# Yachim/schwarzschild-raytracer

Hardware: AMD Instinct MI355X
Metric: Mpixels/s at 1920x1080, 2000 geodesic steps; 1/2/4/8 MI355X (higher is better)
Workload: dtype f32

## Files before the change

### schwarzschild-raytracer_amd/csrc/kernels/geodesic.hip

```cpp
#include <hip/hip_runtime.h>

#include <cstdint>
#include <type_traits>

typedef float sr_v4f __attribute__((ext_vector_type(4)));
typedef const __attribute__((address_space(4))) sr_v4f sr_cfloat4;
__device__ __forceinline__ float4 ldc(const sr_cfloat4* p) {
    const sr_v4f v = *p;
    return make_float4(v.x, v.y, v.z, v.w);
}

#include "../device_scene.h"

namespace {

#define SR_PI 3.1415926535f
#define SR_EPS 0.0000001f

struct f2 { float x, y; };
struct f3 { float x, y, z; };
struct f4 { float x, y, z, w; };
struct m3 { f3 c0, c1, c2; };

__device__ __forceinline__ f2 F2(float x, float y) { f2 r; r.x = x; r.y = y; return r; }
// ... 283 lines not shown
            c = fminf(c - qm, SR_BUDGET_TMAX);
        }
    }
    return c - 1.8f * slot_mu(sl) * a;
}
__device__ __forceinline__ float clearance_bh(float a) {
    return (fabsf(a - 1.0f) - SR_MU_QUADRATIC * 3.0f) - 1.8f * SR_MU_QUADRATIC * a;
}
__device__ __forceinline__ bool outward_clear(float cn, float br, float mu, float qk, float pl1, float a, float dip) {
    const float S = __builtin_fmaf(0.01f * a, a, __builtin_fmaf(2.0f, a, 1.0f));
    const float Sc = S + pl1;
    return a * dip > (cn + br + __builtin_fmaf(mu, S, qk * Sc * Sc)) * 1.001f;
}
__device__ __forceinline__ float plane_window(const sr_dev_slot& sl, f3 A, f3 B, float a, float perr, float dphi) {
    const f3 dv = B - A;
    const f3 nrm_ = ld3(sl.a1);
    const float y = dot(B - ld3(sl.pos), nrm_);
    const float len = __builtin_amdgcn_sqrtf(dot(dv, dv));
    if (!(len > 1e-6f) || !(len < 0.5f * a) || !(a > 1.0f)) return 0.0f;
    const float il = __builtin_amdgcn_rcpf(len);
    const float a2 = a * a;
    const float kap = 6.06f * __builtin_amdgcn_rcpf(a2);
    const float c = (y > 0.0f ? -1.0f : 1.0f) * dot(dv, nrm_) * il;
    const float th0 = __builtin_fmaf(kap, len, __builtin_fmaf(2.0f * perr, il, 1e-4f));
    const float m = (sl.mp + sl.mu * __builtin_fmaf(3.1f, a, 1.0f)) * 1.001f + perr;
    const float R = fabsf(y) - m;
    if (!(R > 0.0f)) return 0.0f;
    const float b = c + th0;
    const float L = (__builtin_amdgcn_sqrtf(__builtin_fmaf(b, b, 2.0f * kap * R)) - b) * (a2 * (1.0f / 6.06f));
    const float ch = 1.5f * a * dphi;
    const float Lc = fminf(L, fminf(__builtin_fmaf(0.5f, a, -ch), (1.5f - th0) * (a2 * (1.0f / 6.06f)) - ch));
    const float th1 = __builtin_fmaf(kap, Lc, th0);
    const float f = 1.0f - (th1 * th1 + th1 * th0 + th0 * th0) * (1.0f / 6.0f);
    return (Lc > 0.0f && f > 0.0f) ? Lc * f * 0.998f : 0.0f;
}
#ifndef SR_INIT_WINDOW
#define SR_INIT_WINDOW 1
#endif
struct PlaneWinCam {
    bool ok;
    f3 wn;
    float k2r;
    float kap, a2s, cap;
};
__device__ __forceinline__ PlaneWinCam plane_window_cam(const sr_dev_slot& sl, f3 A, float a, float perr, float dphi) {
    PlaneWinCam w;
    w.ok = false;
    w.wn = F3(0.0f, 0.0f, 0.0f);
    w.k2r = w.kap = w.a2s = w.cap = 0.0f;
    const f3 nrm_ = ld3(sl.a1);
    const float y = dot(A - ld3(sl.pos), nrm_);
    if (!(a > 1.0f)) return w;
    const float a2 = a * a;
    const float kap = 6.06f * __builtin_amdgcn_rcpf(a2);
    w.wn = nrm_ * (y > 0.0f ? -1.0f : 1.0f);
    const float th0 = 1e-4f;
    const float m = (sl.mp + sl.mu * __builtin_fmaf(3.1f, a, 1.0f)) * 1.001f + perr;
    const float R = fabsf(y) - m;
    if (!(R > 0.0f)) return w;
    w.k2r = 2.0f * kap * R;
    w.kap = kap;
    w.a2s = a2 * (1.0f / 6.06f);
    const float ch = 1.5f * a * dphi;
    w.cap = fminf(__builtin_fmaf(0.5f, a, -ch), (1.5f - th0) * (a2 * (1.0f / 6.06f)) - ch);
    w.ok = true;
    return w;
}
__device__ __forceinline__ float plane_window_dir(f3 wn, float k2r, float kap, float a2s, float cap, f3 d) {
    const float c = dot(d, wn);
    const float th0 = 1e-4f;
    const float b = c + th0;
    const float L = (__builtin_amdgcn_sqrtf(__builtin_fmaf(b, b, k2r)) - b) * a2s;
    const float Lc = fminf(L, cap);
    const float th1 = __builtin_fmaf(kap, Lc, th0);
    const float f = 1.0f - (th1 * th1 + th1 * th0 + th0 * th0) * (1.0f / 6.0f);
    return (Lc > 0.0f && f > 0.0f) ? Lc * f * 0.998f : 0.0f;
}
#ifndef SR_OUT_CYL_CM
#define SR_OUT_CYL_CM 1
#endif
#ifndef SR_OUT_FAR
#define SR_OUT_FAR 1
#endif
__device__ __forceinline__ bool outward_slot(const sr_dev_slot& sl, bool cyl_par, float a, float dip) {
    if (SR_OUT_CYL_CM) cyl_par = false;
    if (sl.type == SR_OBJECT_PLANE || (sl.type == SR_OBJECT_CYLINDER && (cyl_par || !(sl.x1 > 0.0f)))) return false;
    if (SR_OUT_FAR)
        return outward_clear(sl.rf, 0.0f, slot_mu(sl), sl.type == SR_OBJECT_CYLINDER ? sl.qk : 0.0f, sl.pl1, a, dip);
    return outward_clear(sl.cn, sl.br, sl.mu, sl.type == SR_OBJECT_CYLINDER ? sl.qk : 0.0f, sl.pl1, a, dip);
}

#define SR_PIN(x) asm volatile("" : "+s"(x))
__device__ __forceinline__ sr_dev_slot pin_slot(const sr_dev_slot& g) {
    sr_dev_slot sl = g;
    SR_PIN(sl.type);
    SR_PIN(sl.rb);
    SR_PIN(sl.mp);
    SR_PIN(sl.br);
    SR_PIN(sl.mu);
    SR_PIN(sl.pl1);
    SR_PIN(sl.qk);
    SR_PIN(sl.bc[0]);
    SR_PIN(sl.bc[1]);
    SR_PIN(sl.bc[2]);
    SR_PIN(sl.x0);
    SR_PIN(sl.pos[0]);
    SR_PIN(sl.pos[1]);
    SR_PIN(sl.pos[2]);
    SR_PIN(sl.x1);
    SR_PIN(sl.a0[0]);
    SR_PIN(sl.a0[1]);
    SR_PIN(sl.a0[2]);
    SR_PIN(sl.x2);
    SR_PIN(sl.a1[0]);
    SR_PIN(sl.a1[1]);
    SR_PIN(sl.a1[2]);
    SR_PIN(sl.a2[0]);
    SR_PIN(sl.a2[1]);
    SR_PIN(sl.a2[2]);
    return sl;
}

__device__ __forceinline__ float clearance_slab(const sr_dev_slot& sl, f3 A, float a) {
    if (!(sl.mp < INFINITY)) return -INFINITY;
    const float y = dot(A - ld3(sl.pos), ld3(sl.a1));
    const float ey = fmaxf(0.0f, fmaxf(-y, y - sl.x0));
    return ey - sl.mp - 1.8f * SR_MU_QUADRATIC * a;
}

__device__ __forceinline__ float nmin(float m, float e) { return __builtin_elementwise_minimum(m, e); }

#ifndef SR_WG
#define SR_WG 64
#endif
#define SR_WG_PER_TILE (256 / SR_WG)
#define SR_E_STRIDE SR_WG
#ifndef SR_NC_KERNEL
#define SR_NC_KERNEL 0
#endif
#ifndef SR_AHEAD
#define SR_AHEAD 2.0f
#endif
#ifndef SR_FAST_UNROLL
#define SR_FAST_UNROLL SR_FAST_UNROLL_DEFAULT
#endif
#ifndef SR_AHEAD_T
#define SR_AHEAD_T 1.0f
#endif
#ifndef SR_CM_ITER
#define SR_CM_ITER 1
#endif
#ifndef SR_COAST
#define SR_COAST 1
#endif
template <int NB, int NC, bool TR = false>
struct BudgetLayout {
    static constexpr int PA0 = NB + 1;
    static constexpr int SLAB0 = PA0 + 2 * NC;
    static constexpr int BT = SLAB0 + NC;
    static constexpr int BM = BT + 1, BCX = BT + 2, BCY = BT + 3, BMH = BT + 4, BCM = BT + 5, BUHI = BT + 6;
    static constexpr int BTR = BT + 7;
    static constexpr int ROWS = BT + 7 + (TR ? 1 : 0);
};
#define SR_REACH_TR (1u << 30)
#ifndef SR_BH_WINDOW
#define SR_BH_WINDOW 1
#endif
#define SR_BH_U 0.986f
#define SR_U_NOWIN 0x1.93e592p+99f
#define SR_BH_RWIN 1.0143f
#ifndef SR_BH_WINDOW2
#define SR_BH_WINDOW2 1
#endif
#define SR_BH_ULO2 0.90910f
#define SR_BH_RMAX2 1.0999f
#define SR_BH_DIP2 0.9995f
#define SR_BH_DIP 0.9935f

__device__ __forceinline__ float ball_q(float R, float cx, float cy) {
    if (!(R < INFINITY)) return R == INFINITY ? -INFINITY : INFINITY;
    const float c = fabsf(cx) + fabsf(cy);
    const float Rt = R * (1.0f / 1.0101f) - 3.0e-6f * (c + R);
    if (!(Rt > 0.0f)) return INFINITY;
    const float s = c + Rt;
    return __builtin_fmaf(2.0e-6f * s, s, (cx * cx + cy * cy) - Rt * Rt);
}

template <int NB_, int NC_, bool TR_ = false>
struct Budget {
    using L = BudgetLayout<NB_, NC_, TR_>;
    static constexpr int NB = NB_, NC = NC_;
    static constexpr bool TR = TR_;
    float* E;
    __device__ __forceinline__ float ld(int row) const { return E[row * SR_E_STRIDE]; }
    __device__ __forceinline__ void st(int row, float v) const { E[row * SR_E_STRIDE] = v; }
    __device__ __forceinline__ float T() const { return ld(L::BT); }
    __device__ __forceinline__ void setT(float v) const { st(L::BT, v); }
    __device__ __forceinline__ float m() const { return ld(L::BM); }
    __device__ __forceinline__ void setM(float v) const { st(L::BM, v); }
    __device__ __forceinline__ float cx() const { return ld(L::BCX); }
    __device__ __forceinline__ float cy() const { return ld(L::BCY); }
    __device__ __forceinline__ void setC(float x, float y) const {
        st(L::BCX, x);
        st(L::BCY, y);
    }
    __device__ __forceinline__ float mh() const { return ld(L::BMH); }
    __device__ __forceinline__ void setMh(float v) const { st(L::BMH, v); }
    __device__ __forceinline__ uint32_t cm() const { return __float_as_uint(ld(L::BCM)) & 0xffu; }
    __device__ __forceinline__ uint32_t excl() const { return __float_as_uint(ld(L::BCM)) >> 8; }
    __device__ __forceinline__ void setCm(uint32_t cm, uint32_t excl) const {
        st(L::BCM, __uint_as_float(cm | (excl << 8)));
    }
    __device__ __forceinline__ float etr() const { return ld(L::BTR); }
    __device__ __forceinline__ void setEtr(float v) const { st(L::BTR, v); }
    __device__ __forceinline__ float uhi() const { return ld(L::BUHI); }
    __device__ __forceinline__ void setUhi(float v) const { st(L::BUHI, v); }
    static __device__ __forceinline__ bool inner(float uhi) { return uhi > SR_BH_U && uhi < 1.0f; }
    static __device__ __forceinline__ float ulo_of(float uhi, float u_f) { return inner(uhi) ? SR_BH_ULO2 : u_f; }
    SR_PROBE_BUDGET_FIELDS
};

__device__ __forceinline__ float xplane_need(const sr_dev_slot& sl, float xs) {
    if (sl.type == SR_OBJECT_PLANE || sl.type == SR_OBJECT_CYLINDER) return INFINITY;
    return (sl.br + sl.mu * xs) * 1.001f + 1.0e-4f + 1.0e-5f * sl.cn;
}
__device__ __forceinline__ uint32_t plane_off_bit(f3 bc, int j, f3 n, float nn, float need) {
    const float h = dot(bc, n);
    return (uint32_t)(h * h > (need * need) * (nn * 1.0002f)) << j;
}
__device__ __forceinline__ uint32_t xplane_bit(const sr_dev_slot& sl, int j, f3 n, float nn, float xs) {
    return plane_off_bit(ld3(sl.bc), j, n, nn, xplane_need(sl, xs));
}
#ifndef SR_XCYL
#define SR_XCYL 1
#endif
__device__ __forceinline__ uint32_t xcyl_bit(const sr_dev_slot& sl, int j, f3 n, float nn, float need) {
    return plane_off_bit(ld3(sl.bc), j, n, nn, need);
}
__device__ __forceinline__ float orbit_e(float u, float du) {
    return u < 0.6f ? __builtin_fmaf(du, du, u * u * (1.0f - u)) : INFINITY;
}
#ifndef SR_XPERI
#define SR_XPERI 1
#endif
template <class BS>
__device__ __forceinline__ uint32_t budget_cyl_frame(const sr_dev_scene* __restrict__ sc, BS& bs, f3 nv, f3 tv) {
    uint32_t c = (uint32_t)sc->budget_cyl_mask;
    uint32_t cm = 0;
#pragma unroll
    for (int k = 0; k < BS::NC; k++) {
        if (c) {
            const f3 ax = ld3(sc->slots[__builtin_ctz(c)].a1);
            const float pa = dot(nv, ax), pb = dot(tv, ax);
            bs.E[(BS::L::PA0 + 2 * k) * SR_E_STRIDE] = pa;
            bs.E[(BS::L::PA0 + 1 + 2 * k) * SR_E_STRIDE] = pb;
            cm |= (uint32_t)(!(pa * pa + pb * pb < 1.0f - 2.0f * SR_BUDGET_DPMIN - 1.0e-3f)) << k;
            c &= c - 1;
        }
    }
    return cm;
}
template <class BS>
__device__ __forceinline__ void budget_frame(const sr_dev_scene* __restrict__ sc, BS& bs, f3 nv, f3 tv, float xs,
                                             const float* xneed, const float* xperi, float eo) {
    const uint32_t cm = budget_cyl_frame(sc, bs, nv, tv);
    uint32_t x = 0;
#if SR_XPLANE
    {
        const f3 n = cross(nv, tv);
        const float nn = dot(n, n);
        const int nb = sc->num_budget;
        for (int j = 1; j <= nb; j++) {
            x |= xplane_bit(sc->slots[j - 1], j, n, nn, xs);
            if (SR_XCYL && eo <= SR_XCYL_EMAX) x |= xcyl_bit(sc->slots[j - 1], j, n, nn, xneed[j - 1]);
            if (SR_XPERI && eo <= xperi[j - 1]) x |= 1u << j;
        }
    }
#endif
    bs.setCm(cm, x);
}

template <class BS>
__device__ __forceinline__ bool cyl_par_bit(const sr_dev_scene* __restrict__ sc, const BS& bs, int j) {
    const uint32_t cyl = (uint32_t)sc->budget_cyl_mask;
    if (!((cyl >> (j - 1)) & 1u)) return false;
    return (bs.cm() >> __builtin_popcount(cyl & ((1u << (j - 1)) - 1u))) & 1u;
}

__device__ float clearance_tr(const sr_dev_scene* __restrict__ sc, const float* __restrict__ segs, f3 A, bool outward,
                              float a, float dip, float rlen, uint32_t& gm);

__device__ __forceinline__ float bh_start(float a, float dip, bool bh_ok, bool falling, float u2w, float& uhi) {
    float e = clearance_bh(a);
    uhi = SR_U_NOWIN;
    if (SR_BH_WINDOW && bh_ok && a > SR_BH_RWIN) {
        e = INFINITY;
        uhi = SR_BH_U;
    }
    if (SR_BH_WINDOW2 && dip > SR_BH_DIP2 && a * u2w > 1.000001f && a < SR_BH_RMAX2 && (falling || !(a > SR_BH_RWIN))) {
        e = INFINITY;
        uhi = u2w;
    }
    return e;
}

template <class BS>
// ... 1149 lines not shown
    }
    __device__ __forceinline__ float* hit32(uint32_t id, int j) const {
        const uint64_t row = reinterpret_cast<uint64_t>(p + 4 * n + (size_t)j * n * 8);
        uint64_t a, carry;
        asm("v_mad_u64_u32 %0, %1, %2, 32, %3" : "=v"(a), "=s"(carry) : "v"(id), "v"(row));
        return reinterpret_cast<float*>(a);
    }
    __device__ __forceinline__ float& at(int f, size_t id) const { return p[(size_t)(PS_PLANES + f) * n + id]; }
    __device__ __forceinline__ void put3(int f, size_t id, f3 v) const {
        at(f, id) = v.x;
        at(f + 1, id) = v.y;
        at(f + 2, id) = v.z;
    }
    __device__ __forceinline__ f3 get3(int f, size_t id) const { return F3(at(f, id), at(f + 1, id), at(f + 2, id)); }
    __device__ __forceinline__ void puti(int f, size_t id, int v) const { at(f, id) = __int_as_float(v); }
    __device__ __forceinline__ int geti(int f, size_t id) const { return __float_as_int(at(f, id)); }
    __device__ __forceinline__ void put4(int f, size_t id, f4 v) const {
        at(f, id) = v.x;
        at(f + 1, id) = v.y;
        at(f + 2, id) = v.z;
        at(f + 3, id) = v.w;
    }
    __device__ __forceinline__ f4 get4(int f, size_t id) const {
        return F4(at(f, id), at(f + 1, id), at(f + 2, id), at(f + 3, id));
    }
};

__device__ __forceinline__ f4 crosshair_frag(const sr_dev_frame& fr, const Pix& q) {
    f4 frag = F4(0.0f, 0.0f, 0.0f, 0.0f);
    if (fr.crosshair) {
        f2 uv = F2((float)(2 * q.px + 1) / (float)fr.width - 1.0f, (float)(2 * q.py + 1) / (float)fr.height - 1.0f);
        float hx = fabsf(uv.x * fr.res_x / 2.0f), hy = fabsf(uv.y * fr.res_y / 2.0f);
        if ((hx < 1.0f && hy > 5.0f && hy < 15.0f) || (hy < 1.0f && hx > 5.0f && hx < 15.0f))
            frag = F4(0.5f, 0.5f, 0.5f, 0.5f);
    }
    return frag;
}

__device__ __forceinline__ int init_pixel(const sr_dev_frame& fr, const sr_dev_cam& cam, const sr_dev_start& st,
                                          const Pix& q, Ray& r) {
    f2 uv = F2((float)(2 * q.px + 1) / (float)fr.width - 1.0f, (float)(2 * q.py + 1) / (float)fr.height - 1.0f);
    f2 uvv = F2(uv.x, uv.y * fr.res_y / fr.res_x);
    m3 axes = ldm(cam.axes);
    r.ro = ld3(cam.pos);
    r.rd = nrm(mv(axes, F3(uvv.x, uvv.y, cam.ray_forward)));
    r.nv = ld3(st.nv);
    r.steps = 0;
    r.i = 0;
    SR_PROBE(probe_ray_init(r));
    const bool flat = fr.raytrace_type == SR_RAYTRACE_FLAT ||
                      (fr.raytrace_type == SR_RAYTRACE_HALF_WIDTH && uv.x > 2.0f * fr.curved_percentage + -1.0f) ||
                      (fr.raytrace_type == SR_RAYTRACE_HALF_HEIGHT && uv.y > 2.0f * fr.curved_percentage + -1.0f);
    if (flat || fabsf(dot(r.rd, r.nv)) >= 1.0f - SR_EPS) return ST_FLAT;
    if (fr.percent_black >= 0.0f) {
        float x = t_sin(uvv.x * 12.9898f + uvv.y * 78.233f) * 43758.5453f;
        if (x - floorf(x) <= fr.percent_black) return ST_DONE;
    }
    r.tv = nrm(cross(cross(r.nv, r.rd), r.nv));
    r.u = st.u;
    r.du = -r.u * dot(r.rd, r.nv) / dot(r.rd, r.tv);
    return -1;
}

__shared__ uint32_t sr_lds_pid[SR_WG];
struct HitLog {
    PS ps;
    int n;
    __device__ __forceinline__ uint32_t id() const {
        typedef volatile const __attribute__((address_space(3))) uint32_t lds_u32;
        uint32_t t = threadIdx.x;
        asm volatile("" : "+v"(t));
        return *(lds_u32*)&sr_lds_pid[t];
    }
};

__device__ __forceinline__ f3 point_at(const Ray& r, float u, float c, float s) { return (r.nv * c + r.tv * s) / u; }

__device__ __forceinline__ f3 point_near(const Ray& r, float rad, float c, float s) {
    return r.nv * (rad * c) + r.tv * (rad * s);
}

__device__ __forceinline__ float point_err(float rA, float rB) { return 4.0e-6f * (rA + rB); }

__device__ __forceinline__ float ddu(float u) { return -u * (1.0f - 1.5f * u); }

__device__ __forceinline__ float half_step(float a, float q, float h) { return __builtin_fmaf(0.5f, q * h, a); }
__device__ __forceinline__ void rk4_step(float u, float du, float h, float h6, float& un, float& dun) {
    const float k1 = du;
    const float l1 = ddu(u);
    const float k2 = half_step(du, l1, h);
    const float l2 = ddu(half_step(u, k1, h));
    const float k3 = half_step(du, l2, h);
    const float l3 = ddu(half_step(u, k2, h));
    const float k4 = du + l3 * h;
    const float l4 = ddu(u + k3 * h);
    un = u + h6 * (__builtin_fmaf(2.0f, k3, __builtin_fmaf(2.0f, k2, k1)) + k4);
    dun = du + h6 * (__builtin_fmaf(2.0f, l3, __builtin_fmaf(2.0f, l2, l1)) + l4);
}

__device__ __forceinline__ bool flat_misses(const sr_dev_scene* __restrict__ sc, f3 ro, f3 rd) {
    return !sc->tr_visible && dot(ro, rd) >= 0.0f && dot(ro, ro) > sc->flat_miss_r2;
}

__shared__ int sr_lds_ev[SR_WG / 64];

template <bool CULL, bool RECORD, bool WCOST = false, int NB = SR_MAX_BUDGET, int FU = SR_FAST_UNROLL,
          int NC = SR_NC_KERNEL, bool TR = false>
__device__ __forceinline__ int integrate(const sr_dev_scene* __restrict__ sc, const float* __restrict__ segs,
                                         const float4* __restrict__ tbl, const sr_dev_frame& fr, const Tex& tx,
                                         Ray& r, Hit& hit, HitLog& log, const sr_dev_start* __restrict__ start = nullptr) {
    using BS = Budget<NB, NC, TR && CULL>;
    __shared__ float lds_E[BS::L::ROWS * SR_E_STRIDE];
    BS bs;
    bs.E = lds_E + threadIdx.x;
    SR_PROBE(SR_PROF_CLOCK(prof_bi_));
    if (!CULL) bs.setUhi(INFINITY);
    if constexpr (CULL && RECORD)
        budget_start(sc, *start, bs, fr.num_budget, r.ro, r.nv, r.tv, r.du < 0.0f && r.u < 0.6f, r.du > 0.0f,
                     orbit_e(r.u, r.du), r.rd);
    else if (CULL)
        budget_init(sc, segs, bs, r.ro, r.nv, r.tv, r.du < 0.0f && r.u < 0.6f, fr.out_dip,
                    fr.win_ok && fr.out_dip > SR_BH_DIP, r.du > 0.0f, fr.xplane_s, fr.bh_u2, fr.xlow_need,
                    fr.xperi_e, orbit_e(r.u, r.du));
    SR_PROBE(FireProbe<Ray, BS> fire_probe_(r, bs));
    const int N = fr.max_steps;
    const bool every = !CULL || sc->num_step > 0 || (sc->tr_visible && !BS::TR);
    int im = r.i - 1;
    float up = 0.0f;
    float rA = __builtin_amdgcn_rcpf(r.u);
    const int sbase = r.steps - r.i;
    auto phi_cs = [&](int j) -> f2 {
        if (j < 0) return F2(1.0f, 0.0f);
        const float4 t = tbl[j];
        return F2(t.z, t.w);
    };
    auto settle_prev = [&](int i) {
        if (im == i - 1) return;
        const f2 p1 = phi_cs(i - 1);
        f3 A;
        if (im == i - 2) {
            A = r.ro;
        } else {
            const f2 p2 = phi_cs(i - 2);
            A = point_at(r, up, p2.x, p2.y);
        }
        f3 B = point_at(r, r.u, p1.x, p1.y);
        f3 delta = B - A;
        float seg = len(delta);
        r.rd = delta / seg;
        r.ro = B;
        im = i - 1;
    };
    bool force = false;
    int i = r.i;
    SR_PROBE(LoopProbe lp(i); SR_PROF_LOOP_START(r, bs, prof_bi_));
    for (;;) {
        if (RECORD) i = __builtin_amdgcn_readfirstlane(i);
        if (i >= N) break;
        SR_PT(21);
        if (__ballot(r.u < fr.u_f)) {
            if (r.u < fr.u_f) {
                r.i = i;
                r.steps = sbase + i + 1;
                settle_prev(i);
                if (CULL)
                {
                    const float ocx = bs.cx(), ocy = bs.cy();
                    bs.setT(__builtin_fmaf(len(r.ro - (r.nv * ocx + r.tv * ocy)), 1.0101f,
                                           3.0e-6f * (fabsf(ocx) + fabsf(ocy) + 1.0f)));
                }
                float lam;
                if (!sphere_lambda_r2(r.ro, r.rd, F3(0.0f, 0.0f, 0.0f), fr.uf_radius2, -1.0f, lam))
                    return flat_misses(sc, r.ro, r.rd) ? ST_BG : ST_FLAT;
                const f3 q = r.ro + r.rd * lam;
                r.nv = nrm(q);
                if (fabsf(dot(r.rd, r.nv)) >= 1.0f - SR_EPS) return flat_misses(sc, r.ro, r.rd) ? ST_BG : ST_FLAT;
                r.tv = nrm(cross(cross(r.nv, r.rd), r.nv));
                r.u = 1.0f / len(q);
                r.du = -r.u * dot(r.rd, r.nv) / dot(r.rd, r.tv);
                if (CULL) budget_frame(sc, bs, r.nv, r.tv, fr.xplane_s, fr.xlow_need, fr.xperi_e,
                                          orbit_e(r.u, r.du));
                force = true;
            }
            SR_PT(1);
        }
        const float bm = bs.m();
        const float lim0 = (every || force) ? -INFINITY : bm;
        const float uhi = bs.uhi();
        const float ulo = BS::ulo_of(uhi, fr.u_f);
        const float bcx = CULL ? bs.cx() : 0.0f, bcy = CULL ? bs.cy() : 0.0f;
        const float bn = -2.0f * bcx, bt = -2.0f * bcy;
        const float q0 = (!CULL || every || force) ? INFINITY : ball_q(bm, bcx, bcy);
        float vb;
        const uint32_t bcm = CULL ? bs.cm() : 0u;
        const bool any_cm = CULL && NC > 0 && __ballot(bcm != 0u);
        const sr_cfloat4* tp = (const sr_cfloat4*)(tbl + i);
        float4 e;
        float un, dun, rB;
        uint32_t par;
        auto fast = [&](auto cm_tag) {
            constexpr int CMV = decltype(cm_tag)::value;
            constexpr bool CM = CMV != 0;
            par = 0;
            e = ldc(tp);
            f2 pc = CM ? phi_cs(i - 1) : F2(0.0f, 0.0f);
            const CylDirs<NC> cd = CM ? cyl_dirs(sc, bs) : CylDirs<NC>{};
            const float qh = CM ? ((every || force) ? INFINITY : ball_q(nmin(bm, bs.mh()), bcx, bcy)) : q0;
            if (CM) __builtin_amdgcn_s_waitcnt(0xc07f);
            float qit = q0;
            auto compute = [&](int k) -> bool {
                rk4_step(r.u, r.du, e.x, e.y, un, dun);
                float q = q0;
                if (CULL && CMV == 1) {
                    rB = __builtin_amdgcn_rcpf(un);
                    par = chord_parallel(bcm, cd, rB * e.z - rA * pc.x, rB * e.w - rA * pc.y, point_err(rA, rB));
                    q = par ? qh : q0;
                }
                if (CULL && CMV == 2) {
                    if (k == 0) {
                        const float ra = __builtin_amdgcn_rcpf(r.u);
                        rB = __builtin_amdgcn_rcpf(un);
                        par = chord_parallel(bcm, cd, rB * e.z - ra * pc.x, rB * e.w - ra * pc.y, point_err(ra, rB));
                        qit = par ? qh : q0;
                    }
                    q = qit;
                }
                vb = __builtin_fmaf(__builtin_fmaf(q, un, __builtin_fmaf(bt, e.w, bn * e.z)), un, 1.0f);
                SR_STAT(0, 1);
                SR_STAT(13, __popcll(__ballot(1)));
                SR_PROBE(if (CM) SR_STAT_MAIN(31, 1));
                SR_PROBE(if (!(un < 1.0e20f)) SR_TRACE_AT("fast i=%d u=%g un=%g dun=%g vb=%g q=%g\n", i, r.u, un,
                                                            dun, vb, q));
                return __ballot(!(vb < 0.0f) || un < ulo || un > uhi);
            };
            auto apply = [&](float4 en) -> bool {
                r.u = un;
                r.du = dun;
                if (CMV == 1) rA = rB;
                tp += 1;
                if (CM) pc = F2(e.z, e.w);
                e = en;
                return ++i >= N;
            };
            for (;;) {
                float4 nx[FU];
#pragma unroll
                for (int k = 0; k < FU; k++) nx[k] = ldc(tp + 1 + k);
                __builtin_amdgcn_sched_barrier(0);
                bool leave = false;
#pragma unroll
                for (int k = 0; k < FU && !leave; k++) {
                    if (compute(k)) {
#pragma unroll
                        for (int j = k; j < FU; j++) asm volatile("; keep %0" ::"s"(nx[j].x));
                        leave = true;
                    } else {
                        leave = apply(nx[k]);
                    }
                }
                if (leave) break;
            }
        };
        auto coast = [&]() {
            e = ldc(tp);
            for (;;) {
                float4 nx[FU];
#pragma unroll
                for (int k = 0; k < FU; k++) nx[k] = ldc(tp + 1 + k);
                __builtin_amdgcn_sched_barrier(0);
                bool leave = false;
#pragma unroll
                for (int k = 0; k < FU && !leave; k++) {
                    rk4_step(r.u, r.du, e.x, e.y, un, dun);
                    SR_STAT(0, 1);
                    SR_STAT(11, 1);
                    SR_STAT(13, __popcll(__ballot(1)));
                    if (__ballot(!(un >= ulo && un <= uhi))) {
#pragma unroll
                        for (int j = k; j < FU; j++) asm volatile("; keep %0" ::"s"(nx[j].x));
                        leave = true;
                    } else {
                        r.u = un;
                        r.du = dun;
                        tp += 1;
                        e = nx[k];
                        leave = ++i >= N;
                    }
                }
                if (leave) break;
            }
            rA = __builtin_amdgcn_rcpf(r.u);
            rB = __builtin_amdgcn_rcpf(un);
            par = 0;
            vb = -1.0f;
        };
        const int ick = i;
        const float uck = r.u, duck = r.du, upck = up;
        auto recover_up = [&](int ie) -> float {
            if (ie == ick) return upck;
            float u = uck, du = duck;
            for (int j = ick; j < ie - 1; j++) {
                const float4 t0 = tbl[j];
                float un2, dun2;
                rk4_step(u, du, t0.x, t0.y, un2, dun2);
                u = un2;
                du = dun2;
            }
            return u;
        };
        const bool cm_iter = SR_CM_ITER && any_cm && !__ballot(!(uhi < 1.0f)) &&
                             (1.515f * (float)FU) * fr.max_dphi < 0.05f;
        using I0 = std::integral_constant<int, 0>;
        using I1 = std::integral_constant<int, 1>;
        using I2 = std::integral_constant<int, 2>;
        if constexpr (NC > 0) {
            if (cm_iter) fast(I2{});
            else if (any_cm) fast(I1{});
            else if (CULL && SR_COAST && !__ballot(!(lim0 == INFINITY))) coast();
            else fast(I0{});
        } else {
            if (CULL && SR_COAST && !__ballot(!(lim0 == INFINITY))) coast();
            else fast(I0{});
        }
        SR_PT(0);
        if (i >= N) {
            SR_PROBE(SR_STAT_STEPHIST(56, N - 1 - ick); SR_STAT_STEPHIST(57, 1));
            up = recover_up(N);
            break;
        }
        SR_PROBE(SR_PROF_BUMP(r.prof, 19, 1));
        if (CULL && !(r.u < INFINITY) && !(un < INFINITY)) {
            up = r.u;
            break;
        }
        r.i = i;
        r.steps = sbase + i + 1;
        if (un < 0.0f) {
            SR_PROBE(if (i > ick) SR_STAT_STEPHIST(58, i - 1 - ick); SR_STAT_STEPHIST(59, 1));
            up = recover_up(i);
            settle_prev(i);
            return ST_BG;
        }
        const bool bhx = un > uhi || (un < SR_BH_ULO2 && BS::inner(uhi));
        const bool degen = CULL && !(un < 1.0e30f && r.u < 1.0e30f);
        const bool event = !(vb < 0.0f) || bhx || (SR_XPLANE && un < 0.5f * fr.u_f) || degen;
        SR_PROBE(SR_TRACE_AT("slow i=%d u=%.9g un=%.9g uhi=%.9g vb=%g force=%d event=%d bhx=%d m=%g\n", i, r.u, un,
                             uhi, vb, (int)force, (int)event, (int)bhx, bm));
#ifndef SR_BH_CROSS
#define SR_BH_CROSS 1
#endif
        if (RECORD && CULL && SR_BH_CROSS && !every && __ballot(BS::inner(uhi) && un >= SR_BH_UIN3)) {
            const float uin = (uhi == fr.bh_u3 && fr.bh_u3 != fr.bh_u2) ? SR_BH_UIN3 : SR_BH_UIN2;
            if (BS::inner(uhi) && un >= uin && un < 1.0e30f && vb < 0.0f && !force) return ST_BH;
        }
        if (CULL) {
            rA = __builtin_amdgcn_rcpf(r.u);
            rB = __builtin_amdgcn_rcpf(un);
        }
        up = r.u;
        r.u = un;
        r.du = dun;
        const float rAold = rA;
        rA = rB;
        const bool reseeded = force;
        force = false;
        do {
            if (!__ballot(event)) break;
            uint32_t reach = 0xffffffffu;
            uint32_t trmask = 0xffffffffu;
            const f2 p1 = phi_cs(i - 1);
            if (CULL) {
                const bool exact_start = im == i - 1;
                const f3 Ap = exact_start ? r.ro : point_near(r, rAold, p1.x, p1.y);
                const f3 Bp = point_near(r, rB, e.z, e.w);
                const float pe = point_err(exact_start ? 0.0f : rAold, rB);
                float ahead;
                {
                    const float cx = rB * e.z, cy = rB * e.w;
                    const f3 dv = Bp - Ap;
                    const float cl = __builtin_amdgcn_sqrtf(dot(dv, dv));
                    float T;
                    if (reseeded) {
                        T = bs.T() + (cl * 1.0001f + pe) * SR_PATH_SLACK;
                    } else {
                        const float ocx = bs.cx(), ocy = bs.cy();
                        const float dx = cx - ocx, dy = cy - ocy;
                        T = __builtin_fmaf(__builtin_amdgcn_sqrtf(dx * dx + dy * dy), 1.0101f,
                                           3.0e-6f * (rB + fabsf(ocx) + fabsf(ocy)));
                    }
                    bs.setT(T);
                    ahead = SR_AHEAD * SR_PATH_SLACK * cl + SR_AHEAD_T * T;
                    bs.setC(cx, cy);
                }
                SR_STAT(1, 1);
                SR_PROBE(probe_event(sc, bs, r, lp, i, event, vb, q0, bhx, reseeded, ahead, any_cm));
                if (WCOST && (int)__lane_id() == __builtin_ctzll(__ballot(1)))
                    sr_lds_ev[threadIdx.x >> 6] += 1;
                SR_PT(2);
                const bool steep = r.du > 0.0f && __builtin_fmaf(r.du, r.du, r.u * r.u * (1.0f - r.u)) >= SR_BH_E_MIN;
                reach = budget_event(sc, segs, trmask, bs, Ap, Bp, pe, par, reseeded, ahead, r.du < 0.0f && r.u < 0.6f, fr.out_dip,
                                     fr.max_dphi, bhx, fr.win_ok && fr.out_dip > SR_BH_DIP, r.du > 0.0f, cm_iter,
                                     fr.u_f, fr.bh_u2, fr.bh_u3, steep);
                if (__ballot(degen)) {
                    reach |= ((2u << sc->num_budget) - 1u) | SR_REACH_TR;
                    trmask = 0xffffffffu;
                }
                SR_PT(6);
                SR_PROBE(probe_reach(r, reach));
                SR_PROBE(SR_TRACE_AT("  event reach=%x uhi'=%.9g m'=%g E0=%g\n", reach, bs.uhi(), bs.m(), bs.ld(0)));
                if (!__ballot(reach != 0u || every)) break;
                SR_PROBE(probe_fire(bs));
            }
            SR_PROBE(probe_exact_chord(r));
            f3 prev = im == i - 1 ? r.ro : point_at(r, up, p1.x, p1.y);
            r.ro = point_at(r, r.u, e.z, e.w);
            im = i;
            f3 delta = r.ro - prev;
            float seg = len(delta);
            r.rd = delta / seg;
            hit = CULL ? closest_hit_chord<BS::TR>(sc, segs, reach, prev, r.rd, seg, trmask)
                       : closest_hit_all(sc, segs, prev, r.rd, seg);
            SR_PT(4);
            SR_PROBE(SR_TRACE_AT("  chord i=%d seg=%g slot=%d\n", i, seg, hit.slot));
            if (hit.slot != SLOT_NONE) {
                const int op = hit_opacity(sc, fr, tx, hit, -r.rd, !RECORD);
                SR_PT(5);
                if (op == OP_ZERO) break;
                if (!RECORD) return ST_HIT;
                if (hit.slot == SLOT_BH) return ST_BH;
                float4* h = reinterpret_cast<float4*>(
                    log.ps.hit32(log.id(), min((uint32_t)log.n, (uint32_t)(SR_PS_HITS - 1))));
                h[0] = make_float4(hit.p.x, hit.p.y, hit.p.z,
                                   __int_as_float((int)((uint32_t)(hit.slot * 8 + hit.face + PS_KEY_BIAS) |
                                                                  ((uint32_t)r.steps << 8))));
                h[1] = make_float4(r.rd.x, r.rd.y, r.rd.z, hit.p.x);
                log.n++;
                if (op == OP_OPAQUE) return ST_HIT;
                if (log.n == SR_PS_HITS) return ST_MORE;
            }
        } while (false);
        i++;
    }
    r.i = N;
    r.steps = sbase + N;
    settle_prev(N);
    return ST_BG;
}

__device__ __forceinline__ void finish_ray(const sr_dev_scene* __restrict__ sc, const float* __restrict__ segs,
                                           const sr_dev_frame& fr, const Tex& tx, int st, f3 ro, f3 rd, f4& frag) {
    if (st == ST_FLAT) {
        f4 c = intersect_color(sc, segs, fr, tx, ro, rd, -1.0f);
        frag = frag + c;
        if (c.w == 1.0f) return;
        st = ST_BG;
    }
    if (st == ST_BG) frag = frag + get_bg(fr, tx, rd);
}

__device__ __forceinline__ void write_pixel(const sr_dev_frame& fr, uint8_t* __restrict__ out, size_t pitch,
                                            float* __restrict__ dbg_rgba, int32_t* __restrict__ dbg_steps,
                                            const Pix& q, f4 frag, int steps) {
    uint32_t pix = unorm8(frag.x) | (unorm8(frag.y) << 8) | (unorm8(frag.z) << 16) | (unorm8(frag.w) << 24);
    if (out) *reinterpret_cast<uint32_t*>(out + (size_t)q.k * pitch + (size_t)q.px * 4) = pix;
    const size_t i = (size_t)q.k * (size_t)fr.width + (size_t)q.px;
    if (dbg_rgba) {
        dbg_rgba[4 * i + 0] = frag.x;
        dbg_rgba[4 * i + 1] = frag.y;
        dbg_rgba[4 * i + 2] = frag.z;
        dbg_rgba[4 * i + 3] = frag.w;
    }
    if (dbg_steps) dbg_steps[i] = steps;
}

}

#ifndef SR_MIN_WAVES_PER_EU
#define SR_MIN_WAVES_PER_EU 7
#endif
#ifndef SR_NB_SMALL
#define SR_NB_SMALL 6
#endif
#ifndef SR_NC_SMALL
#define SR_NC_SMALL 0
#endif
#ifndef SR_GENERAL_WAVES_PER_EU
#define SR_GENERAL_WAVES_PER_EU 5
#endif
#define SR_NB_GENERAL 8
#define SR_NC_GENERAL SR_NC_KERNEL
#ifndef SR_LARGE_WAVES_PER_EU
#define SR_LARGE_WAVES_PER_EU 5
#endif

constexpr int sr_integrate_waves(int nb, int nc) {
    return nb > SR_NB_GENERAL ? SR_LARGE_WAVES_PER_EU
                              : (nb > SR_NB_SMALL || nc > SR_NC_SMALL) ? SR_GENERAL_WAVES_PER_EU : SR_MIN_WAVES_PER_EU;
}

#define SR_SPLIT 0x80

__device__ __forceinline__ int split_thread(int sub, int tid, int lg) {
    const int lane = tid & 63;
    if (lane >= (1 << lg)) return -1;
    const int cell = sub * 4 + (tid >> 6);
    const int side = lg >> 1;
    const int cpq = 64 >> lg;
    const int quad = cell / cpq, qc = cell % cpq;
    const int per_row = 8 >> side;
    const int x8 = ((qc % per_row) << side) + (lane & ((1 << side) - 1));
    const int y8 = ((qc / per_row) << side) + (lane >> side);
    return quad * 64 + y8 * 8 + x8;
}

__global__ __launch_bounds__(64) void sr_start_table_kernel(const sr_dev_scene* __restrict__ sc,
                                                            const float* __restrict__ segs, sr_dev_frame fr,
                                                            sr_dev_start* __restrict__ start) {
    const int f = (int)blockIdx.x;
    if (f >= fr.batch || threadIdx.x != 0) return;
    build_start(sc, segs, fr, ld3(fr.cam[f].pos), start[f]);
// ... 363 lines not shown
```

### schwarzschild-raytracer_amd/csrc/kernels/probes.h

```cpp
#ifndef SR_PROBES_H
#define SR_PROBES_H

#define SR_STATS_SLOTS 9
#ifdef SR_STATS
__device__ unsigned long long sr_stats[64];
#define SR_WAVE_LOG (1 << 17)
#define SR_WAVE_REC 16
__device__ unsigned long long sr_wave_t[SR_WAVE_REC * SR_WAVE_LOG];
__device__ __forceinline__ void stat_add(int k, unsigned long long v) {
    const unsigned long long act = __ballot(1);
    if ((int)__lane_id() == __builtin_ctzll(act)) atomicAdd(&sr_stats[k], v);
}
#ifdef SR_STATS_NOCOUNT
#define SR_STAT(k, v) ((void)0)
#else
#define SR_STAT(k, v) stat_add(k, v)
#endif
#else
#define SR_STAT(k, v) ((void)0)
#endif

#ifdef SR_LANE_MASK
__device__ const uint8_t* sr_lane_mask;
#endif

#ifdef SR_PROF
#define SR_PROF_N 24
__device__ unsigned long long sr_prof[SR_PROF_N * (1 << 17)];
#define SR_PT(k)                                                      \
    do {                                                              \
        const unsigned t_ = (unsigned)clock64();                      \
        if ((threadIdx.x & 63) == __builtin_ctzll(__ballot(1))) r.prof[k] += t_ - prof_t_; \
        prof_t_ = t_;                                                 \
    } while (0)
#define SR_PTB(k)                                                     \
    do {                                                              \
        const unsigned t_ = (unsigned)clock64();                      \
        if ((threadIdx.x & 63) == __builtin_ctzll(__ballot(1))) bs.prof[k] += t_ - *bs.pt; \
        *bs.pt = t_;                                                  \
    } while (0)
#else
#define SR_PT(k) ((void)0)
#define SR_PTB(k) ((void)0)
#endif

#if defined(SR_STATS) || defined(SR_PROF) || defined(SR_LANE_MASK) || defined(SR_STATS_FIRE)
#define SR_PROBE(...) __VA_ARGS__
#else
#define SR_PROBE(...)
#endif
#ifdef SR_TRACE
#define SR_TRACE_AT(fmt, ...) printf("%c%d " fmt, RECORD ? 'I' : 'R', (int)threadIdx.x, __VA_ARGS__)
#else
#define SR_TRACE_AT(...)
#endif
#define SR_LEAD() ((int)(threadIdx.x & 63) == (int)__builtin_ctzll(__ballot(1)))
#if defined(SR_STATS) && !defined(SR_STATS_BH) && !defined(SR_STATS_DIR)
#define SR_STAT_MAIN(k, v) SR_STAT(k, v)
#else
#define SR_STAT_MAIN(k, v) ((void)0)
#endif
#ifdef SR_STATS_STEPHIST
#define SR_STAT_STEPHIST(k, v) SR_STAT(k, v)
#else
#define SR_STAT_STEPHIST(k, v) ((void)0)
#endif

#ifdef SR_PROF
#define SR_PROF_BUMP(acc, k, v) \
    do {                        \
        if (SR_LEAD()) (acc)[k] += (v); \
    } while (0)
#define SR_PROF_CLOCK(name) const unsigned name = (unsigned)clock64()
#define SR_PROF_LOOP_START(r, bs, t_init)            \
    unsigned prof_t_ = (unsigned)clock64();          \
    (bs).prof = (r).prof;                            \
    (bs).pt = &prof_t_;                              \
    if (SR_LEAD()) (r).prof[22] += prof_t_ - (t_init)
#define SR_PROBE_BUDGET_PROF \
    unsigned* prof;          \
    unsigned* pt;
#define SR_PROBE_RAY_PROF unsigned* prof;
#else
#define SR_PROF_BUMP(acc, k, v) ((void)0)
#define SR_PROF_CLOCK(name) ((void)0)
#define SR_PROF_LOOP_START(r, bs, t_init) ((void)0)
#define SR_PROBE_BUDGET_PROF
#define SR_PROBE_RAY_PROF
#endif
#ifdef SR_STATS_FIRE
#define SR_PROBE_BUDGET_FIRE int fires;
#else
#define SR_PROBE_BUDGET_FIRE
#endif
#ifdef SR_STATS
#define SR_PROBE_RAY_STATS \
    int ev, mat;   \
    int rc[SR_STATS_SLOTS];
#else
#define SR_PROBE_RAY_STATS
#endif
#define SR_PROBE_BUDGET_FIELDS SR_PROBE_BUDGET_FIRE SR_PROBE_BUDGET_PROF
#define SR_PROBE_RAY_FIELDS SR_PROBE_RAY_PROF SR_PROBE_RAY_STATS

template <class R>
__device__ __forceinline__ void probe_ray_init(R& r) {
#ifdef SR_STATS
    r.ev = 0;
    r.mat = 0;
    for (int j = 0; j < SR_STATS_SLOTS; j++) r.rc[j] = 0;
#else
    (void)r;
#endif
}
template <class R>
__device__ __forceinline__ void probe_exact_chord(R& r) {
#ifdef SR_STATS
    r.mat++;
#else
    (void)r;
#endif
}
template <class R>
__device__ __forceinline__ void probe_reach(R& r, uint32_t reach) {
#ifdef SR_STATS
    for (uint32_t c = reach & 0x1ffu; c; c &= c - 1) SR_STAT(2 + __builtin_ctz(c), 1);
#pragma unroll
    for (int j = 0; j < SR_STATS_SLOTS; j++) r.rc[j] += (reach >> j) & 1u;
#else
    (void)r;
    (void)reach;
#endif
}

struct LoopProbe {
#ifdef SR_STATS
    int last_ev, near_run;
    __device__ explicit LoopProbe(int i) : last_ev(i), near_run(0) {}
#else
    __device__ explicit LoopProbe(int) {}
#endif
};
template <class R, class B>
struct FireProbe {
#ifdef SR_STATS_FIRE
    R& r;
    B& b;
    __device__ FireProbe(R& r_, B& b_) : r(r_), b(b_) { b.fires = 0; }
    __device__ ~FireProbe() { r.steps = b.fires; }
#else
    __device__ FireProbe(R&, B&) {}
#endif
};
template <class B>
__device__ __forceinline__ void probe_fire(B& b) {
#ifdef SR_STATS_FIRE
    b.fires++;
#else
    (void)b;
#endif
}
template <class B>
__device__ __forceinline__ void probe_event_phase1(B& bs, float T, float e0, uint32_t forced, uint32_t spent) {
#ifdef SR_PROF
    const unsigned long long b0 = __ballot(!(T < e0) || (forced & 1u));
    if (SR_LEAD()) {
        bs.prof[16] += 1;
        bs.prof[17] += spent == 1u;
        bs.prof[18] += __popcll(b0);
    }
#else
    (void)bs, (void)T, (void)e0, (void)forced, (void)spent;
#endif
}

template <class B, class R>
__device__ __forceinline__ void probe_event(const sr_dev_scene* __restrict__ sc, const B& bs, R& r, LoopProbe& lp,
                                            int i, bool event, float vb, float q0, bool bhx, bool reseeded,
                                            float ahead, bool any_cm) {
#ifdef SR_STATS
    r.ev++;
    {
        const int iv = i - lp.last_ev;
        lp.last_ev = i;
        SR_STAT(32 + (iv <= 1 ? 0 : iv <= 3 ? 1 : iv <= 7 ? 2 : iv <= 15 ? 3 : iv <= 63 ? 4 : 5), 1);
        const int nl = __popcll(__ballot(event));
        SR_STAT(38 + (nl <= 1 ? 0 : nl <= 3 ? 1 : nl <= 7 ? 2 : nl <= 15 ? 3 : nl <= 31 ? 4 : 5), 1);
#if defined(SR_STATS_STEPHIST)
        {
            const int bk = i < 25 ? 0 : i < 100 ? 1 : i < 300 ? 2 : i < 700 ? 3 : i < 1200 ? 4 : 5;
            SR_STAT(44 + bk, 1);
            SR_STAT(50 + bk, nl);
        }
#elif defined(SR_STATS_NEAR)
        {
            const float Tt = bs.T();
            uint32_t sm = 0;
            for (int j = 0; j < 7; j++) {
                const float ej = j <= sc->num_budget ? bs.ld(j) : INFINITY;
                if (__ballot(!(Tt < ej))) sm |= 1u << j;
            }
            const int ns = __popc(sm);
            SR_STAT((iv <= 1 ? 44 : 47) + (ns <= 1 ? 0 : ns == 2 ? 1 : 2), 1);
            if (iv <= 1) {
                lp.near_run++;
                if (ns == 1) SR_STAT(55 + __builtin_ctz(sm), 1);
            } else if (lp.near_run > 0) {
                SR_STAT(50 + (lp.near_run <= 1 ? 0 : lp.near_run <= 3 ? 1 : lp.near_run <= 7 ? 2 : lp.near_run <= 15 ? 3 : 4), 1);
                lp.near_run = 0;
            }
        }
#elif defined(SR_STATS_TRIG)
        {
            const bool ring = r.u > 0.5f && r.u < 0.95f && fabsf(r.du) < 0.15f;
            const float Tt = bs.T();
            for (int j = 0; j < 7; j++) {
                const float ej = j <= sc->num_budget ? bs.ld(j) : INFINITY;
                const bool own = !(Tt < ej);
                SR_STAT(44 + j, __popcll(__ballot(own && ring)));
                SR_STAT(51 + j, __popcll(__ballot(own && !ring)));
                if (j < 6 && __ballot(!(Tt + ahead < ej)) && !__ballot(own)) SR_STAT(58 + j, 1);
            }
        }
#elif defined(SR_STATS_XCYL)
        if (sc->budget_cyl_mask) {
            const int jc = __builtin_ctz((uint32_t)sc->budget_cyl_mask) + 1;
            const sr_dev_slot& sl = sc->slots[jc - 1];
            const float Tt = bs.T();
            uint32_t sm = 0;
            for (int j = 0; j <= sc->num_budget; j++)
                if (__ballot(!(Tt < bs.ld(j)))) sm |= 1u << j;
            const bool own = !(Tt < bs.ld(jc));
            const f3 n = cross(r.nv, r.tv);
            const float h = fabsf(dot(ld3(sl.bc), n)) * __builtin_amdgcn_rsqf(dot(n, n)) - sl.br;
            const float dd[4] = {0.25f, 1.0f, 2.0f, 4.0f};
            SR_STAT(44, __popcll(__ballot(own)));
            if (__ballot(own)) SR_STAT(49, 1);
            if (sm == (1u << jc)) SR_STAT(54, 1);
            for (int k = 0; k < 4; k++) {
                SR_STAT(45 + k, __popcll(__ballot(own && h > dd[k])));
                if (sm == (1u << jc) && !__ballot(own && !(h > dd[k]))) SR_STAT(50 + k, 1);
            }
        }
#else
        if (!__ballot(!(vb < 0.0f))) SR_STAT(44, 1);
        SR_STAT(45, __popcll(__ballot(event && !(q0 < INFINITY))));
        SR_STAT(46, __popcll(__ballot(bhx)));
        SR_STAT(47, nl);
        if (iv <= 1) {
            SR_STAT(48, nl >= 32);
            SR_STAT(49, __popcll(__ballot(event && !(q0 < INFINITY))));
            SR_STAT(50, nl);
            SR_STAT(51, __popcll(__ballot(event && reseeded)));
            SR_STAT(52, __popcll(__ballot(event && bs.m() < 0.05f)));
            SR_STAT(53, any_cm);
            {
                int jm = 0;
                float em = bs.E[0];
                for (int j = 1; j <= sc->num_budget; j++) {
                    const float v = bs.ld(j);
                    if (v < em) { em = v; jm = j; }
                }
                for (int j = 0; j <= 8; j++) SR_STAT(55 + j, __popcll(__ballot(event && jm == j && em < 0.05f)));
            }
        }
        SR_STAT(54, any_cm);
#endif
    }
#endif
#ifdef SR_STATS_BH
    {
        const bool h0 = !(bs.T() < bs.E[0]);
        const bool ring = r.u <= 0.9f && r.u > 0.55f && fabsf(r.du) < 0.1f;
        SR_STAT(23, __popcll(__ballot(h0 && r.u > 1.0f)));
        SR_STAT(24, __popcll(__ballot(h0 && r.u <= 1.0f && r.u > 0.9f)));
        SR_STAT(25, __popcll(__ballot(h0 && ring)));
        SR_STAT(26, __popcll(__ballot(h0 && r.u <= 0.9f && !ring && r.du > 0.0f)));
        SR_STAT(27, __popcll(__ballot(h0 && r.u <= 0.9f && !ring && !(r.du > 0.0f))));
        SR_STAT(28, __popcll(__ballot(event)));
        SR_STAT(29, __popcll(__ballot(h0)));
        SR_STAT(30, __ballot(h0) != 0ull);
        SR_STAT(31, __popcll(__ballot(1)));
    }
#endif
#ifdef SR_STATS_DIR
    {
        const bool outw = r.du < 0.0f && r.u < 0.6f;
        const bool inc = r.du > 0.0f;
        bool any = false;
#pragma unroll
        for (int j = 1; j <= 6; j++) {
            const bool h = !(bs.T() < bs.ld(j));
            any |= h;
            if (j == 3 || j == 5) {
                const int b = j == 3 ? 23 : 26;
                SR_STAT(b, __popcll(__ballot(h && outw)));
                SR_STAT(b + 1, __popcll(__ballot(h && inc)));
                SR_STAT(b + 2, __popcll(__ballot(h && !outw && !inc)));
            }
        }
        SR_STAT(29, __popcll(__ballot(any && outw)));
        SR_STAT(30, __popcll(__ballot(any && inc)));
        SR_STAT(31, __popcll(__ballot(any)));
    }
#endif
    (void)sc, (void)bs, (void)r, (void)lp, (void)i, (void)event, (void)vb, (void)q0, (void)bhx, (void)reseeded;
    (void)ahead, (void)any_cm;
}

#ifdef SR_PROF
__device__ __forceinline__ unsigned* probe_prof_row() {
    __shared__ unsigned prof_lds[4][SR_PROF_N];
    return prof_lds[threadIdx.x >> 6];
}
#endif
struct WaveProbe {
#ifdef SR_STATS
    unsigned long long t_start, c_start, evmat;
    int rcv[SR_STATS_SLOTS];
#endif
#ifdef SR_PROF
    unsigned long long t0;
#endif
    __device__ WaveProbe() {
#ifdef SR_STATS
        t_start = __builtin_amdgcn_s_memrealtime();
        c_start = __builtin_amdgcn_s_memtime();
        evmat = 0;
        for (int j = 0; j < SR_STATS_SLOTS; j++) rcv[j] = 0;
#endif
#ifdef SR_PROF
        if ((threadIdx.x & 63) < SR_PROF_N) probe_prof_row()[threadIdx.x & 63] = 0;
        t0 = clock64();
#endif
    }
    __device__ __forceinline__ int lane_mask(int px, int py, int width, int st, int done) const {
#ifdef SR_LANE_MASK
        if (sr_lane_mask && !sr_lane_mask[(size_t)py * width + px]) return done;
#else
        (void)px, (void)py, (void)width, (void)done;
#endif
        return st;
    }
    template <class R>
    __device__ __forceinline__ void ray_start(R& r) const {
#ifdef SR_PROF
        r.prof = probe_prof_row();
        if (SR_LEAD()) r.prof[23] += (unsigned)(clock64() - t0);
#else
        (void)r;
#endif
    }
    __device__ __forceinline__ void pixel(int st, int n_logged) const {
#if defined(SR_STATS) && !defined(SR_STATS_BH) && !defined(SR_STATS_DIR)
        SR_STAT(23, __popcll(__ballot(1)));
        SR_STAT(24, __popcll(__ballot(n_logged & 1)) + 2 * __popcll(__ballot(n_logged & 2)) +
                        4 * __popcll(__ballot(n_logged & 4)));
        for (int k = 0; k < 6; k++) SR_STAT(25 + k, __popcll(__ballot(st == k)));
#else
        (void)st, (void)n_logged;
#endif
    }
    template <class R>
    __device__ __forceinline__ void ray_end(const R& r) {
#ifdef SR_STATS
        evmat = ((unsigned long long)r.ev << 32) | (unsigned)r.mat;
        for (int j = 0; j < SR_STATS_SLOTS; j++) rcv[j] = r.rc[j];
#else
        (void)r;
#endif
    }
    __device__ __forceinline__ void finish(int frame, int tiles, int block, int ttid, int steps) const {
#ifdef SR_STATS
        {
            int sm = steps;
            unsigned long long em = evmat;
            for (int off = 32; off > 0; off >>= 1) {
                sm = max(sm, __shfl_xor(sm, off));
                const unsigned long long o = __shfl_xor(em, off);
                em = o > em ? o : em;
            }
            int rcm[SR_STATS_SLOTS];
            for (int j = 0; j < SR_STATS_SLOTS; j++) {
                rcm[j] = rcv[j];
                for (int off = 32; off > 0; off >>= 1) rcm[j] = max(rcm[j], __shfl_xor(rcm[j], off));
            }
            const int w = (frame * tiles + block) * 4 + (ttid >> 6);
            if ((threadIdx.x & 63) == 0 && w < SR_WAVE_LOG) {
                unsigned long long* rec = sr_wave_t + (size_t)SR_WAVE_REC * w;
                rec[0] = t_start;
                rec[1] = __builtin_amdgcn_s_memrealtime();
                rec[2] = (unsigned long long)sm;
                rec[3] = em;
                for (int j = 0; j < SR_STATS_SLOTS; j++) rec[4 + j] = (unsigned long long)rcm[j];
                rec[13] = __builtin_amdgcn_s_getreg((3 << 11) | 20);
                rec[14] = __builtin_amdgcn_s_getreg((31 << 11) | 4);
// ... 67 lines not shown
```

Before: 2873.

## Retire or reseed lanes inside the coast loop instead of exiting to slow path

Factors the in-loop reseed into a lambda and, in the RECORD coast path, handles a wave-wide exit from the [ulo,uhi] band in place when no lane needs the full event logic. Lanes that fall below u_f are reseeded or parked with their final status, and parked lanes keep stepping with an unbounded band until the wave leaves. This avoids the costly event and budget processing for coast exits that only need a reseed or retirement. The cost is extra divergence and control complexity, plus parked lanes doing wasted RK4 steps. Probe counters are added for profiling.

```diff
diff --git a/schwarzschild-raytracer_amd/csrc/kernels/geodesic.hip b/schwarzschild-raytracer_amd/csrc/kernels/geodesic.hip
--- a/schwarzschild-raytracer_amd/csrc/kernels/geodesic.hip
+++ b/schwarzschild-raytracer_amd/csrc/kernels/geodesic.hip
@@ -459,6 +459,9 @@
 #endif
 #ifndef SR_COAST
 #define SR_COAST 1
+#endif
+#ifndef SR_RETIRE_COAST
+#define SR_RETIRE_COAST 1
 #endif
 template <int NB, int NC, bool TR = false>
 struct BudgetLayout {
@@ -1914,38 +1917,45 @@
         im = i - 1;
     };
     bool force = false;
+    auto reseed = [&](int i) -> int {
+        r.i = i;
+        r.steps = sbase + i + 1;
+        settle_prev(i);
+        if (CULL)
+        {
+            const float ocx = bs.cx(), ocy = bs.cy();
+            bs.setT(__builtin_fmaf(len(r.ro - (r.nv * ocx + r.tv * ocy)), 1.0101f,
+                                   3.0e-6f * (fabsf(ocx) + fabsf(ocy) + 1.0f)));
+        }
+        float lam;
+        if (!sphere_lambda_r2(r.ro, r.rd, F3(0.0f, 0.0f, 0.0f), fr.uf_radius2, -1.0f, lam))
+            return flat_misses(sc, r.ro, r.rd) ? ST_BG : ST_FLAT;
+        const f3 q = r.ro + r.rd * lam;
+        r.nv = nrm(q);
+        if (fabsf(dot(r.rd, r.nv)) >= 1.0f - SR_EPS) return flat_misses(sc, r.ro, r.rd) ? ST_BG : ST_FLAT;
+        r.tv = nrm(cross(cross(r.nv, r.rd), r.nv));
+        r.u = 1.0f / len(q);
+        r.du = -r.u * dot(r.rd, r.nv) / dot(r.rd, r.tv);
+        if (CULL) budget_frame(sc, bs, r.nv, r.tv, fr.xplane_s, fr.xlow_need, fr.xperi_e,
+                                  orbit_e(r.u, r.du));
+        force = true;
+        return -1;
+    };
+    bool reseeded_in_loop = false;
     int i = r.i;
     SR_PROBE(LoopProbe lp(i); SR_PROF_LOOP_START(r, bs, prof_bi_));
     for (;;) {
         if (RECORD) i = __builtin_amdgcn_readfirstlane(i);
         if (i >= N) break;
         SR_PT(21);
-        if (__ballot(r.u < fr.u_f)) {
+        if (!reseeded_in_loop && __ballot(r.u < fr.u_f)) {
             if (r.u < fr.u_f) {
-                r.i = i;
-                r.steps = sbase + i + 1;
-                settle_prev(i);
-                if (CULL)
-                {
-                    const float ocx = bs.cx(), ocy = bs.cy();
-                    bs.setT(__builtin_fmaf(len(r.ro - (r.nv * ocx + r.tv * ocy)), 1.0101f,
-                                           3.0e-6f * (fabsf(ocx) + fabsf(ocy) + 1.0f)));
-                }
-                float lam;
-                if (!sphere_lambda_r2(r.ro, r.rd, F3(0.0f, 0.0f, 0.0f), fr.uf_radius2, -1.0f, lam))
-                    return flat_misses(sc, r.ro, r.rd) ? ST_BG : ST_FLAT;
-                const f3 q = r.ro + r.rd * lam;
-                r.nv = nrm(q);
-                if (fabsf(dot(r.rd, r.nv)) >= 1.0f - SR_EPS) return flat_misses(sc, r.ro, r.rd) ? ST_BG : ST_FLAT;
-                r.tv = nrm(cross(cross(r.nv, r.rd), r.nv));
-                r.u = 1.0f / len(q);
-                r.du = -r.u * dot(r.rd, r.nv) / dot(r.rd, r.tv);
-                if (CULL) budget_frame(sc, bs, r.nv, r.tv, fr.xplane_s, fr.xlow_need, fr.xperi_e,
-                                          orbit_e(r.u, r.du));
-                force = true;
+                const int st = reseed(i);
+                if (st >= 0) return st;
             }
             SR_PT(1);
         }
+        reseeded_in_loop = false;
         const float bm = bs.m();
         const float lim0 = (every || force) ? -INFINITY : bm;
         const float uhi = bs.uhi();
@@ -2023,38 +2033,79 @@
                 if (leave) break;
             }
         };
-        auto coast = [&]() {
-            e = ldc(tp);
+        auto coast = [&]() -> int {
+            constexpr bool RETIRE = SR_RETIRE_COAST && RECORD;
+            int park = -1;
+            float lo = ulo, hi = uhi;
             for (;;) {
-                float4 nx[FU];
+                e = ldc(tp);
+                for (;;) {
+                    float4 nx[FU];
 #pragma unroll
-                for (int k = 0; k < FU; k++) nx[k] = ldc(tp + 1 + k);
-                __builtin_amdgcn_sched_barrier(0);
-                bool leave = false;
+                    for (int k = 0; k < FU; k++) nx[k] = ldc(tp + 1 + k);
+                    __builtin_amdgcn_sched_barrier(0);
+                    bool leave = false;
 #pragma unroll
-                for (int k = 0; k < FU && !leave; k++) {
-                    rk4_step(r.u, r.du, e.x, e.y, un, dun);
-                    SR_STAT(0, 1);
-                    SR_STAT(11, 1);
-                    SR_STAT(13, __popcll(__ballot(1)));
-                    if (__ballot(!(un >= ulo && un <= uhi))) {
+                    for (int k = 0; k < FU && !leave; k++) {
+                        rk4_step(r.u, r.du, e.x, e.y, un, dun);
+                        SR_STAT(0, 1);
+                        SR_STAT(11, 1);
+                        SR_STAT(13, __popcll(__ballot(1)));
+                        if (__ballot(!(un >= lo && un <= hi))) {
 #pragma unroll
-                        for (int j = k; j < FU; j++) asm volatile("; keep %0" ::"s"(nx[j].x));
-                        leave = true;
-                    } else {
+                            for (int j = k; j < FU; j++) asm volatile("; keep %0" ::"s"(nx[j].x));
+                            leave = true;
+                        } else {
+                            r.u = un;
+                            r.du = dun;
+                            tp += 1;
+                            e = nx[k];
+                            leave = ++i >= N;
+                        }
+                    }
+                    if (leave) break;
+                }
+                if constexpr (RETIRE) {
+                    const bool stays = park < 0 && (un > hi || (un < SR_BH_ULO2 && BS::inner(hi)) ||
+                                                    (SR_XPLANE && un < 0.5f * fr.u_f) ||
+                                                    !(un < 1.0e30f && r.u < 1.0e30f) || un < 0.0f ||
+                                                    (BS::inner(hi) && un >= SR_BH_UIN3));
+                    if (i + 1 < N && !__ballot(stays)) {
+                        SR_PROBE(SR_RETIRE_STAT(1, 1));
+                        up = r.u;
                         r.u = un;
                         r.du = dun;
                         tp += 1;
-                        e = nx[k];
-                        leave = ++i >= N;
+                        ++i;
+                        bool goes_on = false;
+                        if (park < 0 && r.u < fr.u_f) {
+                            const int st = reseed(i);
+                            if (st >= 0) {
+                                park = st | (r.steps << 3);
+                                r.u = 0.0f;
+                                r.du = 0.0f;
+                                lo = -INFINITY;
+                                hi = INFINITY;
+                            } else {
+                                goes_on = true;
+                            }
+                        }
+                        SR_PROBE(SR_RETIRE_STAT(2, __popcll(__ballot(park >= 0 && (park >> 3) == sbase + i + 1))));
+                        if (__ballot(goes_on)) {
+                            SR_PROBE(SR_RETIRE_STAT(3, 1));
+                            reseeded_in_loop = true;
+                        } else if (__ballot(park < 0)) {
+                            continue;
+                        }
                     }
                 }
-                if (leave) break;
+                break;
             }
             rA = __builtin_amdgcn_rcpf(r.u);
             rB = __builtin_amdgcn_rcpf(un);
             par = 0;
             vb = -1.0f;
+            return park;
         };
         const int ick = i;
         const float uck = r.u, duck = r.du, upck = up;
@@ -2075,16 +2126,24 @@
         using I0 = std::integral_constant<int, 0>;
         using I1 = std::integral_constant<int, 1>;
         using I2 = std::integral_constant<int, 2>;
+        int park = -1;
         if constexpr (NC > 0) {
             if (cm_iter) fast(I2{});
             else if (any_cm) fast(I1{});
-            else if (CULL && SR_COAST && !__ballot(!(lim0 == INFINITY))) coast();
+            else if (CULL && SR_COAST && !__ballot(!(lim0 == INFINITY))) park = coast();
             else fast(I0{});
         } else {
-            if (CULL && SR_COAST && !__ballot(!(lim0 == INFINITY))) coast();
+            if (CULL && SR_COAST && !__ballot(!(lim0 == INFINITY))) park = coast();
             else fast(I0{});
         }
         SR_PT(0);
+        if (SR_RETIRE_COAST && RECORD) {
+            if (park >= 0) {
+                r.steps = park >> 3;
+                return park & 7;
+            }
+            if (reseeded_in_loop) continue;
+        }
         if (i >= N) {
             SR_PROBE(SR_STAT_STEPHIST(56, N - 1 - ick); SR_STAT_STEPHIST(57, 1));
             up = recover_up(N);
@@ -2127,7 +2186,10 @@
         const bool reseeded = force;
         force = false;
         do {
-            if (!__ballot(event)) break;
+            if (!__ballot(event)) {
+                SR_PROBE(SR_RETIRE_STAT(0, 1));
+                break;
+            }
             uint32_t reach = 0xffffffffu;
             uint32_t trmask = 0xffffffffu;
             const f2 p1 = phi_cs(i - 1);
diff --git a/schwarzschild-raytracer_amd/csrc/kernels/probes.h b/schwarzschild-raytracer_amd/csrc/kernels/probes.h
--- a/schwarzschild-raytracer_amd/csrc/kernels/probes.h
+++ b/schwarzschild-raytracer_amd/csrc/kernels/probes.h
@@ -25,7 +25,7 @@
 #endif
 
 #ifdef SR_PROF
-#define SR_PROF_N 24
+#define SR_PROF_N 28
 __device__ unsigned long long sr_prof[SR_PROF_N * (1 << 17)];
 #define SR_PT(k)                                                      \
     do {                                                              \
@@ -64,6 +64,17 @@
 #define SR_STAT_STEPHIST(k, v) SR_STAT(k, v)
 #else
 #define SR_STAT_STEPHIST(k, v) ((void)0)
+#endif
+#if defined(SR_STATS_RETIRE)
+#define SR_RETIRE_STAT(k, v) SR_STAT(44 + (k), v)
+#elif defined(SR_PROF)
+#define SR_RETIRE_STAT(k, v)                      \
+    do {                                          \
+        const unsigned v_ = (unsigned)(v);        \
+        if (SR_LEAD()) r.prof[24 + (k)] += v_;    \
+    } while (0)
+#else
+#define SR_RETIRE_STAT(k, v) ((void)0)
 #endif
 
 #ifdef SR_PROF
@@ -242,6 +253,7 @@
                 if (sm == (1u << jc) && !__ballot(own && !(h > dd[k]))) SR_STAT(50 + k, 1);
             }
         }
+#elif defined(SR_STATS_RETIRE)
 #else
         if (!__ballot(!(vb < 0.0f))) SR_STAT(44, 1);
         SR_STAT(45, __popcll(__ballot(event && !(q0 < INFINITY))));
```

After: 2914, median of 6. 1.4% higher.
